# LucasAlegre/morl-baselines

Hardware: NVIDIA H100
Metric: envelope_q_updates_per_sec (higher is better)
Workload: dtype f32

## Files before the change

morl_baselines_b200/csrc/gemm_planes.cu:

```cuda
#include <cuda.h>
#include <cuda_bf16.h>
#include <cuda_fp16.h>
#include <stdlib.h>
#include <string.h>

#include "common.cuh"
#include "gemm_tc.cuh"

namespace morl {

constexpr int kGemmBM = 128;
constexpr int kGemmThreads = 384;
constexpr int kGemmConsumerRegs = 232, kGemmProducerRegs = 40;
constexpr int kGemmBoxN = 32;

__device__ unsigned int g_plane_overflow;


__device__ __forceinline__ void note_overflow(float amax) {
    if (amax > 65504.f) atomicAdd(&g_plane_overflow, 1u);
}

#define MORL_DISPATCH_FMT(F_, ...)                                                         \
    switch (F_) {                                                                          \
// ... 316 lines not shown
                    }
                }
                if (g.drop_bits) {
                    kept |= __shfl_xor_sync(0xffffffffu, kept, 1);
                    kept |= __shfl_xor_sync(0xffffffffu, kept, 2);
                    if (l4 == 0 && row < g.M) g.drop_bits[(size_t)row * relu_bits_words(N) + relu_bits_word(32 * c)] = kept;
                }
            }
        }
    }
    if (!g.ln) return;
    const float inv_n = 1.0f / (float)N;
#pragma unroll
    for (int h = 0; h < 2; ++h) {
        float s = 0.f;
#pragma unroll
        for (int c = 0; c < 8; ++c)
            if (32 * c < N)
#pragma unroll
                for (int t = 0; t < 8; ++t) s = __fadd_rn(s, acc[16 * c + 4 * (t >> 1) + 2 * h + (t & 1)]);
        s = __fadd_rn(s, __shfl_xor_sync(0xffffffffu, s, 1));
        s = __fadd_rn(s, __shfl_xor_sync(0xffffffffu, s, 2));
        const float mean = __fmul_rn(s, inv_n);
        float v = 0.f;
#pragma unroll
        for (int c = 0; c < 8; ++c)
            if (32 * c < N)
#pragma unroll
                for (int t = 0; t < 8; ++t) {
                    const float d = __fsub_rn(acc[16 * c + 4 * (t >> 1) + 2 * h + (t & 1)], mean);
                    v = __fmaf_rn(d, d, v);
                }
        v = __fadd_rn(v, __shfl_xor_sync(0xffffffffu, v, 1));
        v = __fadd_rn(v, __shfl_xor_sync(0xffffffffu, v, 2));
        const float rstd = rsqrtf(__fadd_rn(__fmul_rn(v, inv_n), g.ln_eps));
#pragma unroll
        for (int c = 0; c < 8; ++c)
            if (32 * c < N)
#pragma unroll
                for (int t = 0; t < 8; ++t) {
                    const int col = 32 * c + 8 * (t >> 1) + 2 * l4 + (t & 1);
                    const int j = 16 * c + 4 * (t >> 1) + 2 * h + (t & 1);
                    const float gm = g.ln_gamma ? __ldg(g.ln_gamma + col) : 1.0f, bt = g.ln_beta ? __ldg(g.ln_beta + col) : 0.0f;
                    acc[j] = __fmaf_rn(__fmul_rn(__fsub_rn(acc[j], mean), rstd), gm, bt);
                }
    }
}

__device__ __forceinline__ void reload_bias(float* bias_s, const float* bias, int n_begin, int n_end, float mul) {
    bar_sync_named(1, 256);
    const int col = n_begin + (int)threadIdx.x;
    bias_s[threadIdx.x] = (bias && col < n_end) ? __ldg(bias + col) * mul : 0.f;
    bar_sync_named(1, 256);
}

template <int FMT, int SPLIT, bool PRE, typename AfterMma>
__device__ __forceinline__ void consume_unit(float (&acc)[128], const KSmem& s, Ring& ring, int n_kblk, int n_begin, int n_cnt, int rbase, int wg, int lane,
                                             long long* wait_cycles, AfterMma&& after_mma, const EpiArgs& e, const CUtensorMap* tmC, uint8_t* my_stage,
                                             uint32_t& n_stored, float& amax) {
#define MORL_UNIT(N_) \
    case N_: mma_unit<FMT, N_, SPLIT>(acc, s, ring, n_kblk, wg, lane, wait_cycles); break;
    switch (n_cnt) {
        MORL_UNIT(32) MORL_UNIT(64) MORL_UNIT(96) MORL_UNIT(128)
        default:
            if constexpr (!SPLIT) {
                switch (n_cnt) {
                    MORL_UNIT(160) MORL_UNIT(192) MORL_UNIT(224) MORL_UNIT(256)
                    default: __trap();
                }
            } else {
                __trap();
            }
    }
#undef MORL_UNIT
    after_mma();
#pragma unroll
    for (int c = 0; c < (SPLIT ? 4 : 8); ++c) {
        if (32 * c < n_cnt) {
            float a[16];
#pragma unroll
            for (int j = 0; j < 16; ++j) a[j] = SPLIT ? __fadd_rn(acc[16 * c + j], acc[64 + 16 * c + j]) : acc[16 * c + j];
            epilogue_chunk<FMT, PRE>(a, n_begin + 32 * c, rbase, lane, e, tmC, my_stage, n_stored, amax);
        }
    }
}

template <int FMT, int SPLIT, int EPI = kEpiPlain>
__global__ void __launch_bounds__(kGemmThreads, 1)
gemm_planes_kernel(const __grid_constant__ CUtensorMap tmA, const __grid_constant__ CUtensorMap tmB, const __grid_constant__ CUtensorMap tmC,
                   const GemmArgs g) {
    using L = KPlan<FMT>;
    extern __shared__ uint8_t gsmem_raw[];
    const KSmem s = carve_kplan<FMT>(gsmem_raw, (uint32_t)g.n_stages, g.b_stage);

    const int warp = threadIdx.x >> 5;
    const int lane = threadIdx.x & 31;
    const int BN = g.N_pad;
    const int n_tiles = (g.M + kGemmBM - 1) / kGemmBM;
    const int n_kblk = g.K / PlaneFmt<FMT>::BK;
    constexpr int kUnitN = SPLIT ? 128 : 256;
    const int col_units = (BN + kUnitN - 1) / kUnitN;
    const bool wide = BN > 256;
    const int n_work = n_tiles * col_units;
    auto unit_of = [&](int u, int& tile, int& n_begin, int& n_cnt) {
        tile = u / col_units;
        n_begin = (u - tile * col_units) * kUnitN;
        n_cnt = BN - n_begin < kUnitN ? BN - n_begin : kUnitN;
        if (g.reverse) tile = n_tiles - 1 - tile;
    };

    if (threadIdx.x == 0) {
        init_ring_barriers(s.full, s.empty, (uint32_t)g.n_stages);
        g_mbar_init_fence();
    }
    pdl_enter();
    for (int t = threadIdx.x; t < 256; t += blockDim.x) s.bias[t] = (g.bias && t < g.N) ? g.bias[t] : 0.f;
    __syncthreads();

    if (warp >= 8) {
        warpgroup_reg_dec<kGemmProducerRegs>();
        if (warp == 8 && lane == 0) {
            asm volatile("prefetch.tensormap [%0];" ::"l"(&tmA) : "memory");
            asm volatile("prefetch.tensormap [%0];" ::"l"(&tmB) : "memory");
            Ring ring((uint32_t)g.n_stages);
            long long w_empty = 0;
            for (int u = blockIdx.x; u < n_work; u += gridDim.x) {
                int tile, n_begin, n_cnt;
                unit_of(u, tile, n_begin, n_cnt);
                w_empty += load_unit<FMT>(s, ring, &tmA, &tmB, tile * kGemmBM, n_begin, n_cnt, n_kblk, g.stats != nullptr);
            }
            if (g.stats) atomicAdd(&g.stats[2], (unsigned long long)w_empty);
        }
    } else {
        warpgroup_reg_inc<kGemmConsumerRegs>();
        const int wg = warp >> 2;
        uint8_t* my_stage = s.c + warp * 2 * L::kStageC;
        uint32_t n_stored = 0;
        const float c_mul = ld_scale(g.c_scale);
        const bool folded = EPI == kEpiPlain && g.c_f32 == nullptr;
        const float fold = folded ? c_mul : 1.0f;
        if (warp == 0 && folded)
            for (int t = lane; t < 256; t += 32) s.bias[t] *= fold;
        bar_sync_named(1, 256);
        EpiArgs e;
        e.M = g.M; e.N = g.N;
        e.k_acc = fold / (ld_scale(g.a_scale) * ld_scale(g.b_scale));
        e.c_mul = folded ? 1.0f : c_mul;
        e.bias_s = s.bias; e.relu = g.relu; e.bits_in = g.bits_in; e.bits_out = g.bits_out; e.bits_ld = g.bits_ld; e.mask = g.mask;
        e.ld_mask = g.ld_mask; e.c_f32 = g.c_f32; e.ldc = g.ldc; e.planes = g.c_planes != nullptr; e.ldp = g.ldp;
        uint32_t key0 = 0, key1 = 0, ctr0 = 0;
        if constexpr (EPI == kEpiLn) {
            if (g.drop_seed) {
                const unsigned long long seed = *g.drop_seed;
                key0 = (uint32_t)seed;
                key1 = (uint32_t)(seed >> 32);
                ctr0 = *g.drop_offset;
            }
        }
        float amax = 0.f;
        float acc[128];
        Ring ring((uint32_t)g.n_stages);
        long long w_full = 0, busy = 0;
        const long long t_begin = g.stats ? clock64() : 0;
        for (int u = blockIdx.x; u < n_work; u += gridDim.x) {
            int tile, n_begin, n_cnt;
            unit_of(u, tile, n_begin, n_cnt);
            const int rbase = tile * kGemmBM + wg * 64 + (warp & 3) * 16;
            long long c1 = 0;
            consume_unit<FMT, SPLIT, EPI == kEpiLn>(acc, s, ring, n_kblk, n_begin, n_cnt, rbase, wg, lane, g.stats ? &w_full : nullptr, [&] {
                c1 = g.stats ? clock64() : 0;
                if (wide) {
                    reload_bias(s.bias, g.bias, n_begin, g.N, fold);
                    e.bias_s = s.bias - n_begin;
                }
                if constexpr (EPI == kEpiLn) ln_dropout_unit(acc, n_cnt, rbase, lane, s.bias, e.k_acc, g, key0, key1, ctr0);
            }, e, &tmC, my_stage, n_stored, amax);
            if (g.stats) busy += clock64() - c1;
        }
        if (g.stats && warp == 0 && lane == 0) {
            atomicAdd(&g.stats[0], (unsigned long long)w_full);
            atomicAdd(&g.stats[1], (unsigned long long)(clock64() - t_begin));
            atomicAdd(&g.stats[3], (unsigned long long)busy);
        }
        if (FMT == MORL_FMT_F16X2) note_overflow(amax);
        if (lane == 0) asm volatile("cp.async.bulk.wait_group 0;" ::: "memory");
    }
}

constexpr int kChainMaxJobs = 8;
constexpr int kChainLanes = 4;

struct alignas(64) ChainMaps {
    CUtensorMap A[kChainMaxJobs];
    CUtensorMap B[kChainMaxJobs];
    CUtensorMap C[kChainMaxJobs];
};

struct ChainArgs {
    int M, K;
    int k_first;
    int n_chains, n_layers;
    const float* bias[kChainMaxJobs];
    const float* b_scale[kChainMaxJobs];
    uint32_t* bits_out[kChainMaxJobs];
    const uint32_t* bits_in[kChainMaxJobs];
    const float* a_scale;
    int relu;
    int n_stages;
};

template <int FMT>
__global__ void __launch_bounds__(kGemmThreads, 1)
gemm_chain_kernel(const __grid_constant__ ChainMaps maps, const ChainArgs g) {
    using L = KPlan<FMT>;
    constexpr int BN = 256;
    extern __shared__ uint8_t gsmem_raw[];
    const KSmem s = carve_kplan<FMT>(gsmem_raw, (uint32_t)g.n_stages, L::kBStage);
    uint64_t* stored = s.empty + L::kMaxStages;

    const int warp = threadIdx.x >> 5;
    const int lane = threadIdx.x & 31;
    const int unit = blockIdx.x, n_units = gridDim.x;
    const int n_tiles = (g.M + kGemmBM - 1) / kGemmBM;
    const int n_kblk_full = g.K / PlaneFmt<FMT>::BK, n_kblk_first = g.k_first / PlaneFmt<FMT>::BK;
    const int tiles_per_group = kChainLanes / g.n_chains;
    const int cu0 = unit, cu1 = (unit + n_units / 2) % n_units;
    const int mt0 = cu0 < n_tiles ? (n_tiles - cu0 + n_units - 1) / n_units : 0;
    const int mt1 = g.n_chains > 1 ? (cu1 < n_tiles ? (n_tiles - cu1 + n_units - 1) / n_units : 0) : 0;
    const int n_groups = ((mt0 > mt1 ? mt0 : mt1) + tiles_per_group - 1) / tiles_per_group;
    auto unit_of = [&](int gi, int l, int ln, int& job, int& tile) {
        const int c = ln % g.n_chains, ti = gi * tiles_per_group + ln / g.n_chains;
        job = c * g.n_layers + l;
        tile = ti < (c ? mt1 : mt0) ? (c ? cu1 : cu0) + ti * n_units : -1;
    };

    if (threadIdx.x == 0) {
        init_ring_barriers(s.full, s.empty, (uint32_t)g.n_stages);
        for (int i = 0; i < kChainLanes; ++i) g_mbar_init(&stored[i], 8);
        g_mbar_init_fence();
    }
    pdl_enter();
    __syncthreads();

    if (warp >= 8) {
        warpgroup_reg_dec<kGemmProducerRegs>();
        if (warp == 8 && lane == 0) {
            Ring ring((uint32_t)g.n_stages);
            uint32_t done_on_lane[kChainLanes] = {0u, 0u, 0u, 0u};
            for (int gi = 0; gi < n_groups; ++gi)
                for (int l = 0; l < g.n_layers; ++l)
                    for (int ln = 0; ln < kChainLanes; ++ln) {
                        int job, tile;
                        unit_of(gi, l, ln, job, tile);
                        if (tile < 0) continue;
                        if (l > 0) {
                            g_mbar_wait(&stored[ln], (done_on_lane[ln] - 1u) & 1u);
                            asm volatile("fence.proxy.async.global;" ::: "memory");
                        }
                        ++done_on_lane[ln];
                        load_unit<FMT>(s, ring, &maps.A[job], &maps.B[job], tile * kGemmBM, 0, BN, l == 0 ? n_kblk_first : n_kblk_full, false);
                    }
        }
    } else {
        warpgroup_reg_inc<kGemmConsumerRegs>();
        const int wg = warp >> 2;
        uint8_t* my_stage = s.c + warp * 2 * L::kStageC;
        uint32_t n_stored = 0;
        const float s_act = ld_scale(g.a_scale);
        float amax = 0.f;
        float acc[128];
        Ring ring((uint32_t)g.n_stages);
        for (int gi = 0; gi < n_groups; ++gi)
            for (int l = 0; l < g.n_layers; ++l)
                for (int ln = 0; ln < kChainLanes; ++ln) {
                    int job, tile;
                    unit_of(gi, l, ln, job, tile);
                    if (tile < 0) continue;
                    reload_bias(s.bias, g.bias[job], 0, BN, s_act);
                    EpiArgs e;
                    e.M = g.M; e.N = BN;
                    e.k_acc = s_act / (s_act * ld_scale(g.b_scale[job]));
                    e.c_mul = 1.0f;
                    e.bias_s = s.bias; e.relu = g.relu; e.bits_in = g.bits_in[job]; e.bits_out = g.bits_out[job]; e.bits_ld = relu_bits_words(BN);
                    e.mask = nullptr; e.ld_mask = 0;
                    e.c_f32 = nullptr; e.ldc = 0; e.planes = 1; e.ldp = BN;
                    const int rbase = tile * kGemmBM + wg * 64 + (warp & 3) * 16;
                    consume_unit<FMT, 0, false>(acc, s, ring, l == 0 ? n_kblk_first : n_kblk_full, 0, BN, rbase, wg, lane, nullptr, [] {}, e,
                                                &maps.C[job], my_stage, n_stored, amax);
                    __syncwarp();
                    if (lane == 0) {
                        asm volatile("cp.async.bulk.wait_group 0;" ::: "memory");
                        g_mbar_arrive(&stored[ln]);
                    }
                }
        if (FMT == MORL_FMT_F16X2) note_overflow(amax);
    }
}

struct ResPlan {
    static constexpr int P = 2, BK = 32, kStages = 3;
    static constexpr uint32_t kRowB = BK * 2;
    static constexpr uint32_t kKBlock = P * kGemmBM * kRowB;
    static constexpr uint32_t kPlaneKB = kGemmBM * kRowB;
    static constexpr uint32_t kAct = 8 * kKBlock;
    static constexpr uint32_t kBStage = P * 256 * kRowB;
    static constexpr uint32_t kOffB = kAct;
    static constexpr uint32_t kOffBias = kOffB + kStages * kBStage;
    static constexpr uint32_t kOffBar = kOffBias + 1024;
    static constexpr uint32_t kBytes = kOffBar + 256 + 1024;
    static_assert(kBytes <= 232448, "dynamic shared memory of one CTA on sm_90 (227 KB)");
};

struct alignas(64) ResChainMaps {
    CUtensorMap A[2];
    CUtensorMap B[kChainMaxJobs];
    CUtensorMap C[kChainMaxJobs];
};

struct ResChainArgs {
    int M, K, k_first, n_chains, n_layers;
    const float* bias[kChainMaxJobs];
    const float* b_scale[kChainMaxJobs];
    uint32_t* bits_out[kChainMaxJobs];
    const uint32_t* bits_in[kChainMaxJobs];
    const float* a_scale;
    int relu;
    uint32_t store;
    const float* u[2];
    const float* v[2];
    int W;
    unsigned long long* stats;
};

__device__ __forceinline__ void mma_unit_resident(float (&acc)[128], uint32_t act, const KSmem& s, Ring& ring, int n_kblk, int wg, int lane,
                                                  long long* wait_cycles) {
    using F = PlaneFmt<MORL_FMT_F16X2>;
    using R = ResPlan;
    constexpr uint32_t b_plane = 256u * R::kRowB;
    const uint32_t a_wg = act + (uint32_t)wg * 64u * R::kRowB;
    uint32_t prev = 0;
    for (int kb = 0; kb < n_kblk; ++kb) {
        const long long c0 = wait_cycles ? clock64() : 0;
        g_mbar_wait(&s.full[ring.stage], ring.phase);
        if (wait_cycles) *wait_cycles += clock64() - c0;
        wgmma_fence();
        const uint32_t a0 = a_wg + (uint32_t)kb * R::kKBlock;
        const uint32_t b0 = g_smem_u32(s.b + ring.stage * R::kBStage);
#pragma unroll
        for (int ks = 0; ks < R::BK / 16; ++ks) {
#pragma unroll
            for (int t = 0; t < F::NPROD; ++t) {
                const uint64_t ad = make_desc_k<R::kRowB>(a0 + F::pa(t) * R::kPlaneKB + ks * 32);
                const uint64_t bd = make_desc_k<R::kRowB>(b0 + F::pb(t) * b_plane + ks * 32);
                Wgmma<256>::template mma<MORL_FMT_F16X2, 0, 0>(acc, ad, bd, (kb | ks | t) != 0 ? 1u : 0u);
            }
        }
        wgmma_commit();
        if (kb > 0) {
            wgmma_wait<1>();
            if (lane == 0) g_mbar_arrive(&s.empty[prev]);
        }
        prev = ring.stage;
        ring.advance();
    }
    wgmma_wait<0>();
    if (n_kblk > 0 && lane == 0) g_mbar_arrive(&s.empty[prev]);
}

__device__ __forceinline__ uint8_t* res_chunk(uint8_t* act, int kb, int row, int q) {
    return act + (uint32_t)kb * ResPlan::kKBlock + (uint32_t)row * ResPlan::kRowB + (uint32_t)((q ^ ((row >> 1) & 3)) << 4);
}

__global__ void __launch_bounds__(kGemmThreads, 1)
gemm_chain_resident_kernel(const __grid_constant__ ResChainMaps maps, const ResChainArgs g) {
    using F = PlaneFmt<MORL_FMT_F16X2>;
    using R = ResPlan;
    constexpr int P = R::P, BN = 256;
    extern __shared__ uint8_t gsmem_raw[];
    uint8_t* sm = align_1k(gsmem_raw);
    uint8_t* act = sm;
    KSmem s;
    s.a = nullptr;
    s.b = sm + R::kOffB;
    s.b_stage = R::kBStage;
    s.c = nullptr;
    s.bias = reinterpret_cast<float*>(sm + R::kOffBias);
    s.full = reinterpret_cast<uint64_t*>(sm + R::kOffBar);
    s.empty = s.full + R::kStages;
    uint64_t* act_full = s.empty + R::kStages;
    uint64_t* act_empty = act_full + 1;
    const bool pairs = g.u[0] != nullptr;

    const int warp = threadIdx.x >> 5;
    const int lane = threadIdx.x & 31;
    const int unit = blockIdx.x, n_units = gridDim.x;
    const int n_tiles = (g.M + kGemmBM - 1) / kGemmBM;
    const int n_kblk_full = g.K / R::BK, n_kblk_first = g.k_first / R::BK;
    const int cu0 = unit, cu1 = (unit + n_units / 2) % n_units;
    const int mt0 = cu0 < n_tiles ? (n_tiles - cu0 + n_units - 1) / n_units : 0;
    const int mt1 = g.n_chains > 1 ? (cu1 < n_tiles ? (n_tiles - cu1 + n_units - 1) / n_units : 0) : 0;
    const int n_ti = mt0 > mt1 ? mt0 : mt1;
    auto tile_row = [&](int ti, int c) { return ti < (c ? mt1 : mt0) ? ((c ? cu1 : cu0) + ti * n_units) * kGemmBM : -1; };

    if (threadIdx.x == 0) {
        init_ring_barriers(s.full, s.empty, R::kStages);
        g_mbar_init(act_full, 1);
        g_mbar_init(act_empty, 8);
        g_mbar_init_fence();
    }
    pdl_enter();
    __syncthreads();

    if (warp >= 8) {
        warpgroup_reg_dec<kGemmProducerRegs>();
        if (warp == 8 && lane == 0) {
            Ring ring((uint32_t)R::kStages);
            long long w_empty = 0;
            uint32_t n_in = 0;
            for (int ti = 0; ti < n_ti; ++ti)
                for (int c = 0; c < g.n_chains; ++c) {
                    const int row0 = tile_row(ti, c);
                    if (row0 < 0) continue;
                    for (int l = 0; l < g.n_layers; ++l) {
                        const int job = c * g.n_layers + l;
                        const int nkb = l == 0 ? n_kblk_first : n_kblk_full;
                        for (int kb = 0; kb < nkb; ++kb) {
                            if (!pairs && l == 0 && kb == (nkb < R::kStages ? nkb - 1 : R::kStages - 1)) {
                                if (n_in > 0) {
                                    const long long c0 = g.stats ? clock64() : 0;
                                    g_mbar_wait(act_empty, (n_in - 1u) & 1u);
                                    if (g.stats) w_empty += clock64() - c0;
                                }
                                g_mbar_expect_tx(act_full, (uint32_t)n_kblk_first * R::kKBlock);
                                for (int k = 0; k < n_kblk_first; ++k) tma_load_3d(act + k * R::kKBlock, &maps.A[c], act_full, k * R::BK, row0, 0);
                                ++n_in;
                            }
                            const long long c0 = g.stats ? clock64() : 0;
                            g_mbar_wait(&s.empty[ring.stage], ring.phase ^ 1u);
                            if (g.stats) w_empty += clock64() - c0;
                            uint64_t* full = &s.full[ring.stage];
                            g_mbar_expect_tx(full, R::kBStage);
                            uint8_t* bs = s.b + ring.stage * R::kBStage;
                            for (int p = 0; p < P; ++p) tma_load_3d(bs + (uint32_t)p * 256u * R::kRowB, &maps.B[job], full, kb * R::BK, 0, p);
                            ring.advance();
                        }
                    }
                }
            if (g.stats) atomicAdd(&g.stats[2], (unsigned long long)w_empty);
        }
    } else {
        warpgroup_reg_inc<kGemmConsumerRegs>();
        const int wg = warp >> 2, wr = warp & 3;
        const int l4 = lane & 3, lr = lane >> 2;
        const int trow = wg * 64 + wr * 16;
        const float s_act = ld_scale(g.a_scale);
        const uint32_t act_s = g_smem_u32(act);
        float amax = 0.f;
        float acc[128];
        Ring ring((uint32_t)R::kStages);
        long long w_full = 0, busy = 0, w_act = 0;
        const long long t_begin = g.stats ? clock64() : 0;
        uint32_t n_in = 0;
        for (int ti = 0; ti < n_ti; ++ti)
            for (int c = 0; c < g.n_chains; ++c) {
                const int row0 = tile_row(ti, c);
                if (row0 < 0) continue;
                if (pairs) {
                    if (lane == 0) asm volatile("cp.async.bulk.wait_group.read 0;" ::: "memory");
                    __syncwarp();
                    const float* u = c ? g.u[1] : g.u[0];
                    const float* v = c ? g.v[1] : g.v[0];
#pragma unroll
                    for (int h = 0; h < 2; ++h) {
                        const int rl = trow + lr + 8 * h, row = row0 + rl;
                        const bool ok = row < g.M;
                        const int b = ok ? row / g.W : 0, j = ok ? row - b * g.W : 0;
#pragma unroll 2
                        for (int kb = 0; kb < 8; ++kb) {
                            const int col = kb * 32 + 8 * l4;
                            uint32_t o[P][4];
                            if (ok) {
                                const float4* up = reinterpret_cast<const float4*>(u + (size_t)b * BN + col);
                                const float4* vp = reinterpret_cast<const float4*>(v + (size_t)j * BN + col);
                                const float4 u0 = __ldg(up), u1 = __ldg(up + 1), v0 = __ldg(vp), v1 = __ldg(vp + 1);
                                const float x[8] = {u0.x + v0.x, u0.y + v0.y, u0.z + v0.z, u0.w + v0.w, u1.x + v1.x, u1.y + v1.y, u1.z + v1.z, u1.w + v1.w};
#pragma unroll
                                for (int t = 0; t < 4; ++t) {
                                    uint32_t w[P];
                                    const float r0 = x[2 * t] < 0.f ? 0.f : x[2 * t], r1 = x[2 * t + 1] < 0.f ? 0.f : x[2 * t + 1];
                                    F::split2(r0 * s_act, r1 * s_act, w, amax);
#pragma unroll
                                    for (int p = 0; p < P; ++p) o[p][t] = w[p];
                                }
                            } else {
#pragma unroll
                                for (int t = 0; t < 4; ++t)
#pragma unroll
                                    for (int p = 0; p < P; ++p) o[p][t] = 0u;
                            }
                            uint8_t* dst = res_chunk(act, kb, rl, l4);
#pragma unroll
                            for (int p = 0; p < P; ++p) *reinterpret_cast<uint4*>(dst + p * R::kPlaneKB) = make_uint4(o[p][0], o[p][1], o[p][2], o[p][3]);
                        }
                    }
                    asm volatile("fence.proxy.async.shared::cta;" ::: "memory");
                    bar_sync_named(2 + wg, 128);
                }
                for (int l = 0; l < g.n_layers; ++l) {
                    const int job = c * g.n_layers + l;
                    const bool last = l == g.n_layers - 1, store = (g.store >> job) & 1u;
                    reload_bias(s.bias, g.bias[job], 0, BN, s_act);
                    if (!pairs && l == 0) {
                        const long long c0 = g.stats ? clock64() : 0;
                        g_mbar_wait(act_full, n_in & 1u);
                        if (g.stats) w_act += clock64() - c0;
                    }
                    mma_unit_resident(acc, act_s, s, ring, l == 0 ? n_kblk_first : n_kblk_full, wg, lane, g.stats ? &w_full : nullptr);
                    const long long c1 = g.stats ? clock64() : 0;
                    EpiArgs e;
                    e.M = g.M; e.N = BN;
                    e.k_acc = s_act / (s_act * ld_scale(g.b_scale[job]));
                    e.c_mul = 1.0f;
                    e.bias_s = s.bias; e.relu = g.relu; e.bits_in = g.bits_in[job]; e.bits_out = g.bits_out[job]; e.bits_ld = relu_bits_words(BN);
                    e.mask = nullptr; e.ld_mask = 0; e.c_f32 = nullptr; e.ldc = 0; e.planes = 1; e.ldp = BN;
                    const bool to_tile = !last || store;
                    if (to_tile) {
                        if (lane == 0) asm volatile("cp.async.bulk.wait_group.read 0;" ::: "memory");
                        __syncwarp();
                    }
                    const int rbase = row0 + trow;
#pragma unroll
                    for (int cc = 0; cc < 8; ++cc) {
                        float a[16];
#pragma unroll
                        for (int jj = 0; jj < 16; ++jj) a[jj] = acc[16 * cc + jj];
                        float x[2][8];
                        epilogue_values<false>(a, 32 * cc, rbase, lane, e, x);
                        if (to_tile) {
#pragma unroll
                            for (int h = 0; h < 2; ++h) {
                                const int rl = lr + 8 * h;
#pragma unroll
                                for (int q = 0; q < 4; ++q) {
                                    uint32_t w[P];
                                    F::split2(x[h][2 * q], x[h][2 * q + 1], w, amax);
                                    uint8_t* st = res_chunk(act, cc, trow + rl, q) + 4 * l4;
#pragma unroll
                                    for (int p = 0; p < P; ++p) *reinterpret_cast<uint32_t*>(st + p * R::kPlaneKB) = w[p];
                                }
                            }
                            if (store) {
                                asm volatile("fence.proxy.async.shared::cta;" ::: "memory");
                                __syncwarp();
                                if (lane == 0) {
                                    const uint32_t src = act_s + (uint32_t)cc * R::kKBlock + (uint32_t)trow * R::kRowB;
#pragma unroll
                                    for (int p = 0; p < P; ++p)
                                        asm volatile("cp.async.bulk.tensor.3d.global.shared::cta.bulk_group [%0, {%2, %3, %4}], [%1];" ::"l"(&maps.C[job]),
                                                     "r"(src + p * R::kPlaneKB), "r"(32 * cc), "r"(rbase), "r"(p)
                                                     : "memory");
                                    asm volatile("cp.async.bulk.commit_group;" ::: "memory");
                                }
                            }
                        }
                    }
                    if (!last) {
                        asm volatile("fence.proxy.async.shared::cta;" ::: "memory");
                        bar_sync_named(2 + wg, 128);
                    } else if (!pairs) {
                        __syncwarp();
                        if (lane == 0) {
                            asm volatile("cp.async.bulk.wait_group.read 0;" ::: "memory");
                            g_mbar_arrive(act_empty);
                        }
                    }
                    if (g.stats) busy += clock64() - c1;
                }
                ++n_in;
            }
        if (g.stats && warp == 0 && lane == 0) {
            atomicAdd(&g.stats[0], (unsigned long long)w_full);
            atomicAdd(&g.stats[1], (unsigned long long)(clock64() - t_begin));
            atomicAdd(&g.stats[3], (unsigned long long)busy);
            atomicAdd(&g.stats[4], (unsigned long long)w_act);
        }
        note_overflow(amax);
        if (lane == 0) asm volatile("cp.async.bulk.wait_group 0;" ::: "memory");
    }
}

constexpr int kMnKT = 32;

__device__ __forceinline__ uint64_t make_desc_mn_sw128(uint32_t smem_addr, uint32_t lbo_bytes) {
    uint64_t d = 0;
    d |= (uint64_t)((smem_addr >> 4) & 0x3FFF);
    d |= (uint64_t)((lbo_bytes >> 4) & 0x3FFF) << 16;
    d |= (uint64_t)(1024 >> 4) << 32;
    d |= (uint64_t)1 << 62;
    return d;
}

struct GemmMnArgs {
    int M;
    int n_tiles;
    int NB;
    int rows_per_split;
    float* partial;
    float* colsum_partial;
};

template <int FMT, int NB, bool COLSUM>
__device__ __forceinline__ void mma_mn_unit(const GemmMnArgs& g, int split, int row, int col0, uint8_t* smA, uint8_t* smB, uint32_t a_stage, uint32_t b_stage,
                                            uint32_t chunk_bytes, uint64_t ones_desc, int n_kblk, uint64_t* full, uint64_t* empty, int wg, int lane) {
    using F = PlaneFmt<FMT>;
    constexpr int P = F::P;
    constexpr uint32_t plane = kMnKT * 128u;
    float acc[NB / 2], cs[8];
#pragma unroll
    for (int i = 0; i < NB / 2; ++i) acc[i] = 0.f;
#pragma unroll
    for (int i = 0; i < 8; ++i) cs[i] = 0.f;
    uint32_t stage = 0, phase = 0, prev = 0;
    for (int kb = 0; kb < n_kblk; ++kb) {
        g_mbar_wait(&full[stage], phase);
        wgmma_fence();
        const uint32_t a0 = g_smem_u32(smA + stage * a_stage) + (uint32_t)wg * chunk_bytes;
        const uint32_t b0 = g_smem_u32(smB + stage * b_stage);
#pragma unroll
        for (int ks = 0; ks < kMnKT / 16; ++ks) {
#pragma unroll
            for (int t = 0; t < F::NPROD; ++t) {
                const uint64_t ad = make_desc_mn_sw128(a0 + F::pa(t) * plane + ks * 2048u, chunk_bytes);
                const uint64_t bd = make_desc_mn_sw128(b0 + F::pb(t) * plane + ks * 2048u, chunk_bytes);
                Wgmma<NB>::template mma<FMT, 1, 1>(acc, ad, bd, (kb | ks | t) != 0 ? 1u : 0u);
            }
            if constexpr (COLSUM) {
#pragma unroll
                for (int pl = P - 1; pl >= 0; --pl)
                    Wgmma<16>::template mma<FMT, 1, 1>(cs, make_desc_mn_sw128(a0 + pl * plane + ks * 2048u, chunk_bytes), ones_desc,
                                                       (kb | ks | (P - 1 - pl)) != 0 ? 1u : 0u);
            }
        }
        wgmma_commit();
        if (kb > 0) {
            wgmma_wait<1>();
            if (lane == 0) g_mbar_arrive(&empty[prev]);
        }
        prev = stage;
        if (++stage == (uint32_t)F::kStagesMn) {
            stage = 0;
            phase ^= 1u;
        }
    }
    wgmma_wait<0>();
    const int l4 = lane & 3;
#pragma unroll
    for (int h = 0; h < 2; ++h) {
        float* prow = g.partial + ((size_t)split * g.n_tiles * 128 + row + 8 * h) * g.NB + col0 + 2 * l4;
#pragma unroll
        for (int j = 0; j < NB / 8; ++j) *reinterpret_cast<float2*>(prow + 8 * j) = make_float2(acc[4 * j + 2 * h], acc[4 * j + 2 * h + 1]);
        if (COLSUM && l4 == 0) g.colsum_partial[(size_t)split * g.n_tiles * 128 + row + 8 * h] = cs[2 * h];
    }
}

template <int FMT>
__global__ void __launch_bounds__(kGemmThreads, 1)
gemm_planes_mn_kernel(const __grid_constant__ CUtensorMap tmA, const __grid_constant__ CUtensorMap tmB, const GemmMnArgs g) {
    using F = PlaneFmt<FMT>;
    constexpr int P = F::P;
    constexpr int kStages = F::kStagesMn;
    extern __shared__ uint8_t gsmem_raw[];
    uint8_t* gsmem = align_1k(gsmem_raw);
    constexpr uint32_t chunk_bytes = (uint32_t)P * kMnKT * 128u;
    constexpr uint32_t a_stage = 2u * chunk_bytes;
    constexpr uint32_t b_stage = 4u * chunk_bytes;
    const int k_units = g.NB > 256 ? 2 : 1;
    const int col0 = (int)(blockIdx.x / g.n_tiles % k_units) * 256;
    const int nb = g.NB - col0 < 256 ? g.NB - col0 : 256;
    const int nb_chunks = nb / 64;
    uint8_t* smA = gsmem;
    uint8_t* smB = gsmem + kStages * a_stage;
    uint64_t* full = reinterpret_cast<uint64_t*>(smB + kStages * b_stage);
    uint64_t* empty = full + kStages;
    uint8_t* ones_b = reinterpret_cast<uint8_t*>(empty + kStages);
    uint32_t* ones = reinterpret_cast<uint32_t*>(align_1k(ones_b));
    for (int t = threadIdx.x; t < 1024; t += blockDim.x) ones[t] = F::kOnes2;
    asm volatile("fence.proxy.async.shared::cta;" ::: "memory");

    const int warp = threadIdx.x >> 5, lane = threadIdx.x & 31;
    const int nt = blockIdx.x % g.n_tiles;
    const int split = blockIdx.x / (g.n_tiles * k_units);
    const int m_begin = split * g.rows_per_split;
    const int m_end = min(g.M, m_begin + g.rows_per_split);
    const int n_kblk = (m_end - m_begin + kMnKT - 1) / kMnKT;

    if (threadIdx.x == 0) {
        init_ring_barriers(full, empty, kStages);
        g_mbar_init_fence();
    }
    __syncthreads();
    pdl_enter();

    if (warp >= 8) {
        warpgroup_reg_dec<kGemmProducerRegs>();
        if (warp == 8 && lane == 0) {
            uint32_t stage = 0, phase = 0;
            for (int kb = 0; kb < n_kblk; ++kb) {
                g_mbar_wait(&empty[stage], phase ^ 1u);
                g_mbar_expect_tx(&full[stage], (2u + (uint32_t)nb_chunks) * chunk_bytes);
                const int m0 = m_begin + kb * kMnKT;
                for (int c = 0; c < 2; ++c) tma_load_3d(smA + stage * a_stage + c * chunk_bytes, &tmA, &full[stage], nt * 128 + c * 64, m0, 0);
                for (int c = 0; c < nb_chunks; ++c) tma_load_3d(smB + stage * b_stage + c * chunk_bytes, &tmB, &full[stage], col0 + c * 64, m0, 0);
                if (++stage == kStages) {
                    stage = 0;
                    phase ^= 1u;
                }
            }
        }
    } else {
        warpgroup_reg_inc<kGemmConsumerRegs>();
        const int wg = warp >> 2;
        const uint64_t ones_desc = make_desc_mn_sw128(g_smem_u32(ones), chunk_bytes);
        const bool colsum = g.colsum_partial != nullptr && col0 == 0;
        const int row = nt * 128 + wg * 64 + (warp & 3) * 16 + (lane >> 2);
#define MORL_UNIT(N_)                                                                                                                               \
    case N_:                                                                                                                                        \
        if (colsum) mma_mn_unit<FMT, N_, true>(g, split, row, col0, smA, smB, a_stage, b_stage, chunk_bytes, ones_desc, n_kblk, full, empty, wg, lane); \
        else mma_mn_unit<FMT, N_, false>(g, split, row, col0, smA, smB, a_stage, b_stage, chunk_bytes, ones_desc, n_kblk, full, empty, wg, lane);       \
        break;
        switch (nb) {
            MORL_UNIT(64) MORL_UNIT(128) MORL_UNIT(192) MORL_UNIT(256)
            default: __trap();
        }
#undef MORL_UNIT
    }
}

__global__ void __launch_bounds__(256) reduce_partials_kernel(const float* __restrict__ partial, int S, int prow, int pcol, int rows, int cols,
                                                              int transpose, float* __restrict__ out, int ld_out, int main_blocks,
                                                              const float* __restrict__ vec_partial, float* __restrict__ vec_out,
                                                              const float* __restrict__ scale_a, const float* __restrict__ scale_b) {
    pdl_enter();
    __shared__ float red[8][33];
    float mul = 1.0f / (ld_scale(scale_a) * ld_scale(scale_b));
    if ((int)blockIdx.x >= main_blocks) {
        partial = vec_partial;
        out = vec_out;
        pcol = 1; cols = 1; transpose = 0; ld_out = 1;
        mul = 1.0f / ld_scale(scale_a);
    }
    const int e = ((int)blockIdx.x >= main_blocks ? (int)blockIdx.x - main_blocks : (int)blockIdx.x) * 32 + threadIdx.x;
    const int total = rows * cols;
    float acc = 0.f;
    int r = 0, c = 0;
    if (e < total) {
        r = e / cols;
        c = e - r * cols;
        const float* p = partial + (size_t)r * pcol + c;
        const size_t stride = (size_t)prow * pcol;
        float a0 = 0.f, a1 = 0.f;
        int s = threadIdx.y;
        for (; s + 8 < S; s += 16) {
            a0 += p[(size_t)s * stride];
            a1 += p[(size_t)(s + 8) * stride];
        }
        if (s < S) a0 += p[(size_t)s * stride];
        acc = a0 + a1;
    }
    red[threadIdx.y][threadIdx.x] = acc;
    __syncthreads();
    if (threadIdx.y == 0 && e < total) {
        float t = red[0][threadIdx.x];
#pragma unroll
        for (int y = 1; y < 8; ++y) t += red[y][threadIdx.x];
        t *= mul;
        if (transpose)
            out[(size_t)c * ld_out + r] = t;
        else
            out[(size_t)r * ld_out + c] = t;
    }
}

__global__ void __launch_bounds__(256) reduce_partials_vec4_kernel(const float* __restrict__ partial, int S, int prow, int pcol, int rows, int cols,
                                                                   float* __restrict__ out, int ld_out, int main_blocks,
                                                                   const float* __restrict__ vec_partial, float* __restrict__ vec_out,
                                                                   const float* __restrict__ scale_a, const float* __restrict__ scale_b) {
    pdl_enter();
    __shared__ float4 red[8][33];
    if ((int)blockIdx.x >= main_blocks) {
        const float mul = 1.0f / ld_scale(scale_a);
        const int e = ((int)blockIdx.x - main_blocks) * 32 + threadIdx.x;
        float acc = 0.f;
        if (e < rows) {
            const float* p = vec_partial + e;
            float a0 = 0.f, a1 = 0.f;
            int s = threadIdx.y;
            for (; s + 8 < S; s += 16) {
                a0 += p[(size_t)s * prow];
                a1 += p[(size_t)(s + 8) * prow];
            }
            if (s < S) a0 += p[(size_t)s * prow];
            acc = a0 + a1;
        }
        red[threadIdx.y][threadIdx.x].x = acc;
        __syncthreads();
        if (threadIdx.y == 0 && e < rows) {
            float t = red[0][threadIdx.x].x;
#pragma unroll
            for (int y = 1; y < 8; ++y) t += red[y][threadIdx.x].x;
            vec_out[e] = t * mul;
        }
        return;
    }
    const float mul = 1.0f / (ld_scale(scale_a) * ld_scale(scale_b));
    const int e4 = ((int)blockIdx.x * 32 + threadIdx.x) * 4;
    const int total = rows * cols;
    float4 acc = make_float4(0.f, 0.f, 0.f, 0.f);
    int r = 0, c = 0;
    if (e4 < total) {
        r = e4 / cols;
        c = e4 - r * cols;
        const float* p = partial + (size_t)r * pcol + c;
        const size_t stride = (size_t)prow * pcol;
        constexpr int kRedMax = 12;
        float4 a0 = acc, a1 = acc;
        if (S <= 8 * kRedMax) {
            float4 v[kRedMax];
#pragma unroll
            for (int k = 0; k < kRedMax; ++k) {
                const int sk = threadIdx.y + 8 * k;
                v[k] = sk < S ? __ldcg(reinterpret_cast<const float4*>(p + (size_t)sk * stride)) : make_float4(0.f, 0.f, 0.f, 0.f);
            }
#pragma unroll
            for (int k = 0; k < kRedMax; ++k) {
                if ((int)threadIdx.y + 8 * k < S) {
                    if (k & 1) { a1.x += v[k].x; a1.y += v[k].y; a1.z += v[k].z; a1.w += v[k].w; }
                    else       { a0.x += v[k].x; a0.y += v[k].y; a0.z += v[k].z; a0.w += v[k].w; }
                }
            }
        } else {
            int s = threadIdx.y;
            for (; s + 8 < S; s += 16) {
                const float4 u = *reinterpret_cast<const float4*>(p + (size_t)s * stride);
                const float4 v = *reinterpret_cast<const float4*>(p + (size_t)(s + 8) * stride);
                a0.x += u.x; a0.y += u.y; a0.z += u.z; a0.w += u.w;
                a1.x += v.x; a1.y += v.y; a1.z += v.z; a1.w += v.w;
            }
            if (s < S) {
                const float4 u = *reinterpret_cast<const float4*>(p + (size_t)s * stride);
                a0.x += u.x; a0.y += u.y; a0.z += u.z; a0.w += u.w;
            }
        }
        acc = make_float4(a0.x + a1.x, a0.y + a1.y, a0.z + a1.z, a0.w + a1.w);
    }
    red[threadIdx.y][threadIdx.x] = acc;
    __syncthreads();
    if (threadIdx.y == 0 && e4 < total) {
        float4 t = red[0][threadIdx.x];
#pragma unroll
        for (int y = 1; y < 8; ++y) {
            const float4 q = red[y][threadIdx.x];
            t.x += q.x; t.y += q.y; t.z += q.z; t.w += q.w;
        }
        *reinterpret_cast<float4*>(out + (size_t)r * ld_out + c) = make_float4(t.x * mul, t.y * mul, t.z * mul, t.w * mul);
    }
}

template <int FMT>
__global__ void __launch_bounds__(256) colsum_planes_kernel(const uint16_t* __restrict__ planes, long long plane_stride, int M, int ld, int N,
                                                            int rows_per_chunk, float* __restrict__ part) {
    using F = PlaneFmt<FMT>;
    __shared__ float red[8][32][9];
    const int n0 = (blockIdx.y * 32 + threadIdx.x) * 8;
    const int m0 = blockIdx.x * rows_per_chunk, m1 = min(M, m0 + rows_per_chunk);
    float acc[8];
#pragma unroll
// ... 965 lines not shown
```

Before: 825.2.

## Split resident activation tile barriers per k-block for finer-grained load/release overlap

Replaces the single full/empty barrier pair that guarded the whole resident input tile with one pair per k-block. The producer now issues B-ring loads before the activation loads and refills each activation k-block as soon as it is released. Consumers wait per k-block inside the MMA loop and release k-blocks progressively during the store epilogue, using a lag of outstanding bulk stores. The aim is to overlap loading the next tile's activations with the current tile's tail epilogue and the first MMAs. The cost is more barrier traffic and more complex parity tracking, which could introduce ordering hazards.

```diff
diff --git a/morl_baselines_b200/csrc/gemm_planes.cu b/morl_baselines_b200/csrc/gemm_planes.cu
--- a/morl_baselines_b200/csrc/gemm_planes.cu
+++ b/morl_baselines_b200/csrc/gemm_planes.cu
@@ -642,13 +642,16 @@
     static constexpr uint32_t kRowB = BK * 2;
     static constexpr uint32_t kKBlock = P * kGemmBM * kRowB;
     static constexpr uint32_t kPlaneKB = kGemmBM * kRowB;
-    static constexpr uint32_t kAct = 8 * kKBlock;
+    static constexpr int kActKBlocks = 8;
+    static constexpr int kReleaseLag = 3;
+    static constexpr uint32_t kAct = kActKBlocks * kKBlock;
     static constexpr uint32_t kBStage = P * 256 * kRowB;
     static constexpr uint32_t kOffB = kAct;
     static constexpr uint32_t kOffBias = kOffB + kStages * kBStage;
     static constexpr uint32_t kOffBar = kOffBias + 1024;
     static constexpr uint32_t kBytes = kOffBar + 256 + 1024;
     static_assert(kBytes <= 232448, "dynamic shared memory of one CTA on sm_90 (227 KB)");
+    static_assert((2 * kStages + 2 * kActKBlocks) * 8 <= 256, "ring and input-tile barriers");
 };
 
 struct alignas(64) ResChainMaps {
@@ -673,13 +676,18 @@
 };
 
 __device__ __forceinline__ void mma_unit_resident(float (&acc)[128], uint32_t act, const KSmem& s, Ring& ring, int n_kblk, int wg, int lane,
-                                                  long long* wait_cycles) {
+                                                  long long* wait_cycles, uint64_t* act_full, uint32_t act_parity, long long* act_wait_cycles) {
     using F = PlaneFmt<MORL_FMT_F16X2>;
     using R = ResPlan;
     constexpr uint32_t b_plane = 256u * R::kRowB;
     const uint32_t a_wg = act + (uint32_t)wg * 64u * R::kRowB;
     uint32_t prev = 0;
     for (int kb = 0; kb < n_kblk; ++kb) {
+        if (act_full) {
+            const long long c0 = act_wait_cycles ? clock64() : 0;
+            g_mbar_wait(&act_full[kb], act_parity);
+            if (act_wait_cycles) *act_wait_cycles += clock64() - c0;
+        }
         const long long c0 = wait_cycles ? clock64() : 0;
         g_mbar_wait(&s.full[ring.stage], ring.phase);
         if (wait_cycles) *wait_cycles += clock64() - c0;
@@ -728,7 +736,7 @@
     s.full = reinterpret_cast<uint64_t*>(sm + R::kOffBar);
     s.empty = s.full + R::kStages;
     uint64_t* act_full = s.empty + R::kStages;
-    uint64_t* act_empty = act_full + 1;
+    uint64_t* act_empty = act_full + R::kActKBlocks;
     const bool pairs = g.u[0] != nullptr;
 
     const int warp = threadIdx.x >> 5;
@@ -744,8 +752,10 @@
 
     if (threadIdx.x == 0) {
         init_ring_barriers(s.full, s.empty, R::kStages);
-        g_mbar_init(act_full, 1);
-        g_mbar_init(act_empty, 8);
+        for (int k = 0; k < R::kActKBlocks; ++k) {
+            g_mbar_init(&act_full[k], 1);
+            g_mbar_init(&act_empty[k], 8);
+        }
         g_mbar_init_fence();
     }
     pdl_enter();
@@ -765,16 +775,6 @@
                         const int job = c * g.n_layers + l;
                         const int nkb = l == 0 ? n_kblk_first : n_kblk_full;
                         for (int kb = 0; kb < nkb; ++kb) {
-                            if (!pairs && l == 0 && kb == (nkb < R::kStages ? nkb - 1 : R::kStages - 1)) {
-                                if (n_in > 0) {
-                                    const long long c0 = g.stats ? clock64() : 0;
-                                    g_mbar_wait(act_empty, (n_in - 1u) & 1u);
-                                    if (g.stats) w_empty += clock64() - c0;
-                                }
-                                g_mbar_expect_tx(act_full, (uint32_t)n_kblk_first * R::kKBlock);
-                                for (int k = 0; k < n_kblk_first; ++k) tma_load_3d(act + k * R::kKBlock, &maps.A[c], act_full, k * R::BK, row0, 0);
-                                ++n_in;
-                            }
                             const long long c0 = g.stats ? clock64() : 0;
                             g_mbar_wait(&s.empty[ring.stage], ring.phase ^ 1u);
                             if (g.stats) w_empty += clock64() - c0;
@@ -783,6 +783,18 @@
                             uint8_t* bs = s.b + ring.stage * R::kBStage;
                             for (int p = 0; p < P; ++p) tma_load_3d(bs + (uint32_t)p * 256u * R::kRowB, &maps.B[job], full, kb * R::BK, 0, p);
                             ring.advance();
+                            if (!pairs && l == 0 && kb == (nkb < R::kStages ? nkb - 1 : R::kStages - 1)) {
+                                for (int k = 0; k < n_kblk_first; ++k) {
+                                    if (n_in > 0) {
+                                        const long long c0 = g.stats ? clock64() : 0;
+                                        g_mbar_wait(&act_empty[k], (n_in - 1u) & 1u);
+                                        if (g.stats) w_empty += clock64() - c0;
+                                    }
+                                    g_mbar_expect_tx(&act_full[k], R::kKBlock);
+                                    tma_load_3d(act + k * R::kKBlock, &maps.A[c], &act_full[k], k * R::BK, row0, 0);
+                                }
+                                ++n_in;
+                            }
                         }
                     }
                 }
@@ -850,12 +862,8 @@
                     const int job = c * g.n_layers + l;
                     const bool last = l == g.n_layers - 1, store = (g.store >> job) & 1u;
                     reload_bias(s.bias, g.bias[job], 0, BN, s_act);
-                    if (!pairs && l == 0) {
-                        const long long c0 = g.stats ? clock64() : 0;
-                        g_mbar_wait(act_full, n_in & 1u);
-                        if (g.stats) w_act += clock64() - c0;
-                    }
-                    mma_unit_resident(acc, act_s, s, ring, l == 0 ? n_kblk_first : n_kblk_full, wg, lane, g.stats ? &w_full : nullptr);
+                    mma_unit_resident(acc, act_s, s, ring, l == 0 ? n_kblk_first : n_kblk_full, wg, lane, g.stats ? &w_full : nullptr,
+                                      (!pairs && l == 0) ? act_full : nullptr, n_in & 1u, g.stats ? &w_act : nullptr);
                     const long long c1 = g.stats ? clock64() : 0;
                     EpiArgs e;
                     e.M = g.M; e.N = BN;
@@ -900,6 +908,10 @@
                                                      "r"(src + p * R::kPlaneKB), "r"(32 * cc), "r"(rbase), "r"(p)
                                                      : "memory");
                                     asm volatile("cp.async.bulk.commit_group;" ::: "memory");
+                                    if (last && !pairs && cc >= R::kReleaseLag) {
+                                        asm volatile("cp.async.bulk.wait_group.read %0;" ::"n"(R::kReleaseLag) : "memory");
+                                        g_mbar_arrive(&act_empty[cc - R::kReleaseLag]);
+                                    }
                                 }
                             }
                         }
@@ -911,7 +923,7 @@
                         __syncwarp();
                         if (lane == 0) {
                             asm volatile("cp.async.bulk.wait_group.read 0;" ::: "memory");
-                            g_mbar_arrive(act_empty);
+                            for (int k = store ? R::kActKBlocks - R::kReleaseLag : 0; k < R::kActKBlocks; ++k) g_mbar_arrive(&act_empty[k]);
                         }
                     }
                     if (g.stats) busy += clock64() - c1;
```

Result: no change. 832.2 (median of 6 runs) (+0.8%).
